# petabi/petal-neighbors

Hardware: AMD Instinct MI355X
Metric: exact k-NN queries/sec (1M x 128 fp32, k=10) (higher is better)
Workload: dtype f32; 1 GPU; c2: 1000000 points x 128 dims f32, 10000 queries, k=10, uniform[0,1); n_points=1000000, dim=128, n_queries=10000, k=10, engine=bf16, exchange=none (one shard), rccl_world_size=1

## Files before the change

### petal-neighbors_amd/csrc/bf16_filter.hip

```cpp
#include "pn_internal.h"
#include "topk_buffer.h"

namespace pn {

typedef __bf16 bf16x8 __attribute__((ext_vector_type(8)));
typedef float f32x16 __attribute__((ext_vector_type(16)));
typedef uint32_t u32x4 __attribute__((ext_vector_type(4)));
typedef __attribute__((address_space(3))) void lds_void_b;
typedef const __attribute__((address_space(1))) void glb_void_b;

#ifdef PN_DIAG_BF_COUNT
__device__ unsigned long long g_bfdbg[16];
#define BF_COUNT(i, v) (dbg_[i] += (unsigned long long)(v))
#define BF_DBG_DECL unsigned long long dbg_[12] = {0, 0, 0, 0, 0, 0, 0, 0, 0, 0, 0, 0}
#define BF_DBG_ARG , unsigned long long (&dbg_)[12]
#define BF_DBG_PASS , dbg_
#define BF_DBG_FLUSH(lane)                                                        \
    do {                                                                          \
        if ((lane) == 0)                                                          \
            for (int i_ = 0; i_ < 12; ++i_) {                                     \
                atomicAdd(&g_bfdbg[i_], dbg_[i_]);                                \
                dbg_[i_] = 0;                                                     \
            }                                                                     \
    } while (0)
__device__ __forceinline__ unsigned long long bf_stamp() {
    unsigned long long t;
    asm volatile("s_memtime %0\n\ts_waitcnt lgkmcnt(0)" : "=s"(t)::"memory");
    return t;
}
__device__ __forceinline__ unsigned long long bf_stamp_nw() {
    unsigned long long t;
    asm volatile("s_memtime %0" : "=s"(t));
    return t;
}
__device__ __forceinline__ void bf_settle(unsigned long long &t) { asm volatile("s_waitcnt lgkmcnt(0)" : "+s"(t)::"memory"); }
#else
#define BF_COUNT(i, v) ((void)0)
#define BF_DBG_DECL ((void)0)
#define BF_DBG_ARG
#define BF_DBG_PASS
#define BF_DBG_FLUSH(lane) ((void)0)
#endif

constexpr int kBQ = 256;
constexpr int kBP = 64;
constexpr double kG = 1.0 / 8192.0;
constexpr double kUp = 1.0 + 1.0 / 1099511627776.0;
__host__ __device__ inline int bf16_extra_col(int dim) {
    const int room = (dim + 15) / 16 * 16 - dim;
    return room >= 5 && dim > 16 ? dim : (dim + 15) / 16 * 16;
}
__host__ __device__ inline int bf16_steps(int dim) { return (bf16_extra_col(dim) + 5 + 15) / 16; }
__host__ __device__ inline bool bf16_ci_dim(int dim) { return dim >= 17 && dim <= 128 && bf16_steps(dim) > (dim + 15) / 16; }
__host__ __device__ inline int bf16_steps_for(int dim, bool ci) { return ci ? (dim + 15) / 16 : bf16_steps(dim); }
// ... 708 lines not shown
    const float a = lo3(l0, l1, l2), am = md3(l0, l1, l2);
    const float b = lo3(l3, l4, l5), bm = md3(l3, l4, l5);
    mn = fminf(a, b);
    const float sec_lo = lo3(fmaxf(a, b), am, bm);
    const float dmin = fminf(lo3(d0, d1, d2), fminf(d3, d4));
    sec = fminf(sec_lo, dmin);
    (void)big;
}

template <int KS, bool CI>
__device__ __forceinline__ void bf_chain(const char *arow, const bf16x8 (&pre)[kLA], const bf16x8 (&b0)[KS],
                                         const bf16x8 (&b1)[KS], const f32x16 &c0, f32x16 &w0, f32x16 &w1, f32x16 &r0,
                                         f32x16 &r1, float &m0, float &m1) {
    bf16x8 f[KS];
#pragma unroll
    for (int i = 0; i < kLA && i < KS; ++i) f[i] = pre[i];
    f32x16 z;
#pragma unroll
    for (int i = 0; i < 16; ++i) z[i] = 0.0f;
#pragma unroll
    for (int ks = 0; ks < KS; ++ks) {
        if (ks + kLA < KS) f[ks + kLA] = *reinterpret_cast<const bf16x8 *>(arow + 32 * (ks + kLA));
        if (CI) {
            w0 = __builtin_amdgcn_mfma_f32_32x32x16_bf16(f[ks], b0[ks], ks ? w0 : c0, 0, 0, 0);
            w1 = __builtin_amdgcn_mfma_f32_32x32x16_bf16(f[ks], b1[ks], ks ? w1 : c0, 0, 0, 0);
        } else {
            w0 = __builtin_amdgcn_mfma_f32_32x32x16_bf16(f[ks], b0[ks], ks ? w0 : z, 0, 0, 0);
            w1 = __builtin_amdgcn_mfma_f32_32x32x16_bf16(f[ks], b1[ks], ks ? w1 : z, 0, 0, 0);
        }
#pragma unroll
        for (int i = 16 * ks / KS; i < 16 * (ks + 1) / KS; ++i) {
            m0 = i ? fminf(m0, r0[i]) : r0[0];
            m1 = i ? fminf(m1, r1[i]) : r1[0];
        }
        __builtin_amdgcn_sched_barrier(0);
    }
}

template <int CP>
__device__ __forceinline__ f32x16 bf_cinit(const char *tb, int blk, int h) {
    typedef float f32x4_ __attribute__((ext_vector_type(4)));
    f32x16 c;
#pragma unroll
    for (int g = 0; g < 4; ++g) {
        const f32x4_ v = *reinterpret_cast<const f32x4_ *>(tb + ((blk * 8 + 2 * g + h) * CP + (CP - 1)) * 16);
        c[4 * g + 0] = v[0];
        c[4 * g + 1] = v[1];
        c[4 * g + 2] = v[2];
        c[4 * g + 3] = v[3];
    }
    return c;
}

template <int KS, bool CI, int CP>
__device__ __forceinline__ void bf_chain_p(const char *arow, bf16x8 (&pre)[kLA], const bf16x8 (&b0)[KS],
                                           const bf16x8 (&b1)[KS], f32x16 &c, f32x16 &w0, f32x16 &w1, f32x16 &r0,
                                           f32x16 &r1, float &m0, float &m1, const char *narow, const char *ntb,
                                           int nblk, int h) {
    typedef float f32x4_ __attribute__((ext_vector_type(4)));
    bf16x8 f[KS];
#pragma unroll
    for (int i = 0; i < kLA && i < KS; ++i) f[i] = pre[i];
    f32x16 z, nc = c;
#pragma unroll
    for (int i = 0; i < 16; ++i) z[i] = 0.0f;
#pragma unroll
    for (int ks = 0; ks < KS; ++ks) {
        if (ks + kLA < KS) f[ks + kLA] = *reinterpret_cast<const bf16x8 *>(arow + 32 * (ks + kLA));
#pragma unroll
        for (int i = 0; i < kLA; ++i)
            if (ks == (KS - kLA + i > 0 ? KS - kLA + i : 0))
                pre[i] = *reinterpret_cast<const bf16x8 *>(narow + 32 * (i < KS ? i : 0));
        if (CI) {
#pragma unroll
            for (int g = 0; g < 4; ++g)
                if (ks == (KS - 4 + g > 0 ? KS - 4 + g : 0)) {
                    const f32x4_ v =
                        *reinterpret_cast<const f32x4_ *>(ntb + ((nblk * 8 + 2 * g + h) * CP + (CP - 1)) * 16);
                    nc[4 * g + 0] = v[0];
                    nc[4 * g + 1] = v[1];
                    nc[4 * g + 2] = v[2];
                    nc[4 * g + 3] = v[3];
                }
            w0 = __builtin_amdgcn_mfma_f32_32x32x16_bf16(f[ks], b0[ks], ks ? w0 : c, 0, 0, 0);
            w1 = __builtin_amdgcn_mfma_f32_32x32x16_bf16(f[ks], b1[ks], ks ? w1 : c, 0, 0, 0);
            if (ks == 0) asm volatile("" ::"v"(c));
        } else {
            w0 = __builtin_amdgcn_mfma_f32_32x32x16_bf16(f[ks], b0[ks], ks ? w0 : z, 0, 0, 0);
            w1 = __builtin_amdgcn_mfma_f32_32x32x16_bf16(f[ks], b1[ks], ks ? w1 : z, 0, 0, 0);
        }
#pragma unroll
        for (int i = 16 * ks / KS; i < 16 * (ks + 1) / KS; ++i) {
            m0 = i ? fminf(m0, r0[i]) : r0[0];
            m1 = i ? fminf(m1, r1[i]) : r1[0];
        }
        __builtin_amdgcn_sched_barrier(0);
    }
    c = nc;
}

constexpr uint32_t kShPeriod = 32;
constexpr uint32_t kShMaxPass = 1u << 14;
__device__ __forceinline__ uint32_t sh_load(const uint32_t *p) {
    return __hip_atomic_load(p, __ATOMIC_RELAXED, __HIP_MEMORY_SCOPE_AGENT);
}
__device__ __forceinline__ void sh_store(uint32_t *p, uint32_t v) {
    __hip_atomic_store(p, v, __ATOMIC_RELAXED, __HIP_MEMORY_SCOPE_AGENT);
}
__device__ __forceinline__ void sh_store_entry(uint2 *p, uint32_t key, uint32_t row) {
    __hip_atomic_store(reinterpret_cast<unsigned long long *>(p), ((unsigned long long)row << 32) | key, __ATOMIC_RELAXED,
                       __HIP_MEMORY_SCOPE_AGENT);
}
__device__ __forceinline__ uint32_t sh_tag(uint32_t epoch, uint32_t ncomp) { return (epoch << 20) | ((ncomp & 0xFFu) << 12); }

template <int M>
__device__ __forceinline__ void bf_refresher(const uint2 *__restrict__ cand, const uint32_t *pcnt, uint32_t *gtau,
                                          const uint32_t *done, uint32_t n_main, size_t nq_pad, uint32_t nseg,
                                          uint32_t epoch, uint32_t rank, uint32_t wv, uint32_t n_wv, int lane) {
    constexpr uint32_t CAP = 64u * M;
    constexpr int NK = 8;
// ... 875 lines not shown
                bf_slow<M, false, SH>(a0, p, tau, cnt, rt * kBP, h, jq, lane, kp, ceq, ce_blk, ns BF_DBG_PASS, pc_blk,
                                      &sh_ncomp, sh.epoch);
            cur = nxt;
        }
        if (SH) {
            if (g_pending) tau = fminf(tau, s2f(g0));
        }
        {
            float m = a1[0];
#pragma unroll
            for (int i = 1; i < 16; ++i) m = fminf(m, a1[i]);
            if (__any(m < tau))
                bf_slow<M, false, SH>(a1, m, tau, cnt, (rt1 - 1) * kBP + 32, h, jq, lane, kp, ceq, ce_blk, ns BF_DBG_PASS,
                                      pc_blk, &sh_ncomp, sh.epoch);
            if (SH) {
                if (h == 0) sh_store(pc_blk + jq, sh_tag(sh.epoch, sh_ncomp + 1u));
            }
        }
        asm volatile("s_waitcnt vmcnt(0)" ::: "memory");
        const uint32_t kfin = keep_arg > kp ? keep_arg : kp;
        unsigned long long need = __ballot(h == 0 && cnt > kfin);
        constexpr int NB = M == 1 ? 4 : 1;
        while (need) {
            int jj[NB];
            uint32_t cj[NB], key[NB][M], ixs[NB][M];
#pragma unroll
            for (int bb = 0; bb < NB; ++bb) {
                jj[bb] = need ? __builtin_ctzll(need) : -1;
                if (need) need &= need - 1;
                cj[bb] = jj[bb] >= 0 ? (uint32_t)__builtin_amdgcn_readlane((int)cnt, jj[bb] >= 0 ? jj[bb] : 0) : 0u;
                if (jj[bb] >= 0) bf_compact_load<M>(ce_blk + (size_t)jj[bb] * CAP, cj[bb], lane, key[bb], ixs[bb]);
            }
#pragma unroll
            for (int bb = 0; bb < NB; ++bb) {
                if (jj[bb] >= 0) {
                    uint32_t T, nn;
                    bf_compact_finish<M>(ce_blk + (size_t)jj[bb] * CAP, key[bb], ixs[bb], cj[bb], kp, lane, T, nn);
                    if (jq == jj[bb]) { tau = fminf(tau, s2f(T)); cnt = nn; }
                }
            }
        }
        if (h == 0) {
            ccnt[cell0 + jq] = cnt;
            ctau[cell0 + jq] = f2s(tau);
        }
        BF_DBG_FLUSH(lane);
    }
    if (SH) {
        __syncthreads();
        if (tid == 0) (void)__hip_atomic_fetch_add(sh.done, 1u, __ATOMIC_RELAXED, __HIP_MEMORY_SCOPE_AGENT);
    }
}

template <int M, bool RAD>
__global__ __launch_bounds__(512, 1) void bf16_wide_kernel(const char *__restrict__ img, uint32_t n_tiles,
                                                           const char *__restrict__ Bimg, uint32_t nkc,
                                                           uint32_t tile_bytes, uint32_t has_x, uint32_t kp,
                                                           uint2 *__restrict__ cand, uint32_t *__restrict__ ccnt,
                                                           uint32_t *__restrict__ ctau, size_t nq_pad,
                                                           uint32_t scout_max,
                                                           const uint32_t *__restrict__ tau_init,
                                                           float *__restrict__ scout_out) {
    constexpr uint32_t CAP = 64u * M;
    extern __shared__ __attribute__((aligned(16))) unsigned char smem_raw[];
    char *lds = reinterpret_cast<char *>(smem_raw);

    const int tid = threadIdx.x, lane = tid & 63;
    const int wave = __builtin_amdgcn_readfirstlane(tid >> 6);
    const int jq = lane & 31, h = lane >> 5;
    const int qg = wave & 3, rh = wave >> 2;
    BF_DBG_DECL;

    uint32_t w = blockIdx.x;
    const uint32_t W = gridDim.x;
    {
        const uint32_t x = blockIdx.x & 7u, base = W >> 3, rem = W & 7u;
        w = x * base + (x < rem ? x : rem) + (blockIdx.x >> 3);
    }
    const unsigned long long U = (unsigned long long)(nq_pad / kWR) * n_tiles, Wn = W;
    unsigned long long u0 = (unsigned long long)w * U / Wn;
    const unsigned long long u1 = (unsigned long long)(w + 1) * U / Wn;
    const float inf = __uint_as_float(0x7F800000u);

    int slot_off[4];
#pragma unroll
    for (int s = 0; s < 4; ++s) slot_off[s] = (int)(((unsigned)(2 * s + h) ^ bf_wide_swz((size_t)jq)) * 16u);
    int st = 0;
    uint32_t ns = 0;
    f32x16 acc[4][2];

    while (u0 < u1) {
    const uint32_t qt = (uint32_t)(u0 / n_tiles);
    const unsigned long long v_begin = (unsigned long long)qt * n_tiles, v_end = v_begin + n_tiles;
    const unsigned long long run_end = u1 < v_end ? u1 : v_end;
    const uint32_t rt0 = (uint32_t)(u0 - v_begin), rt1 = (uint32_t)(run_end - v_begin);
    unsigned long long wf = v_begin * Wn / U;
    while ((wf + 1) * U / Wn <= v_begin) ++wf;
    while (wf > 0 && wf * U / Wn > v_begin) --wf;
    const uint32_t sg = (uint32_t)(w - wf);
    const size_t q0 = (size_t)qt * kWR + (size_t)qg * 64;
    const size_t cell0 = (size_t)(sg * 2 + rh) * nq_pad + q0;
    float tau0 = inf, tau1 = inf;
    uint32_t cnt0 = 0, cnt1 = 0;

    const bool is_a = wave < 4;
    const char *src0 = (is_a ? img : Bimg + (size_t)qt * tile_bytes) + (size_t)(wave & 3) * (kWDma * 1024) + lane * 16;
// ... 414 lines not shown
    if (smp) sm = *smp;
    if (sm.seed_out && (!sm.m1 || !sm.a || !sm.b)) return hipErrorInvalidValue;
    if (!bf16_is_wide(dim)) {
        hipLaunchKernelGGL(bf16_pack_queries8_kernel<T>, dim3((unsigned)(nq_pad * 8 / 256)), dim3(256), 0, s, Q, mu, nq,
                           nq_pad, dim, ld, bf16_ks_for(dim, ci), static_cast<uint16_t *>(B), qn, qbad, ci ? 1 : 0,
                           bmax, dmax, Qp, ldq, misc, sm);
        return hipGetLastError();
    }
    if (ci || nq_pad % 32 != 0) return hipErrorInvalidValue;
    hipLaunchKernelGGL((bf16_pack_wide8_kernel<T, true>), dim3((unsigned)(nq_pad * 8 / 256)), dim3(256), 0, s, Q, mu, nq, nq_pad,
                       dim, ld, static_cast<uint16_t *>(B), qn, qbad, (uint32_t *)nullptr, sm);
    return hipGetLastError();
}
template <typename T>
__global__ void bf16_column_moments_kernel(const T *__restrict__ P, const float *__restrict__ mu, size_t n, int dim, size_t ld,
                                           double *__restrict__ out) {
    const size_t r0 = (size_t)blockIdx.x * 1024;
    const size_t r1 = r0 + 1024 < n ? r0 + 1024 : n;
    for (int k = threadIdx.x; k < dim; k += blockDim.x) {
        const double m = (double)mu[k];
        double s1 = 0.0, s2 = 0.0, s3 = 0.0, s4 = 0.0;
        for (size_t r = r0; r < r1; ++r) {
            const double x = (double)P[r * ld + k];
            const double u = (fabs(x) < 1.0e30) ? x - m : 0.0;
            const double u2 = u * u;
            s1 += u;
            s2 += u2;
            s3 += u2 * u;
            s4 += u2 * u2;
        }
        atomicAdd(&out[k], s1);
        atomicAdd(&out[dim + k], s2);
        atomicAdd(&out[2 * dim + k], s3);
        atomicAdd(&out[3 * dim + k], s4);
    }
}
template <typename T>
hipError_t launch_bf16_column_moments(const T *P, const float *mu, size_t n, int dim, size_t ld, double *out, hipStream_t s) {
    hipLaunchKernelGGL(bf16_column_moments_kernel<T>, dim3((unsigned)((n + 1023) / 1024)), dim3(128), 0, s, P, mu, n, dim, ld, out);
    return hipGetLastError();
}
template hipError_t launch_bf16_column_moments<float>(const float *, const float *, size_t, int, size_t, double *, hipStream_t);
template hipError_t launch_bf16_column_moments<double>(const double *, const float *, size_t, int, size_t, double *, hipStream_t);

template hipError_t launch_bf16_pack_queries<float>(const float *, const float *, size_t, size_t, int, size_t, void *, double *,
                                                    uint32_t *, bool, double, double, hipStream_t, float *, size_t, uint32_t *,
                                                    const Bf16SeedModel *);
template hipError_t launch_bf16_pack_queries<double>(const double *, const float *, size_t, size_t, int, size_t, void *, double *,
                                                     uint32_t *, bool, double, double, hipStream_t, double *, size_t, uint32_t *,
                                                     const Bf16SeedModel *);

constexpr uint32_t kBf8MaxRun = 200;
constexpr size_t kBf8MaxImage = (size_t)768 << 20;
template <int KS, int M, bool RAD, bool CI>
static hipError_t launch_bf16_t(const void *img, uint32_t n_tiles, const void *B, uint32_t q_tiles, uint32_t kp,
                                const CandBuf &cb, int n_wg, uint32_t split, uint32_t spp, uint32_t scout_max,
                                const uint32_t *tau_init, float *scout_out, const Bf16Shared *shp, hipStream_t s) {
    const size_t sh = (size_t)3 * kBP * (2 * KS + 1) * 16 + 16;
    const uint32_t kp_keep = kp | ((uint32_t)(M <= 2 && !RAD && cb.final_keep > (int)kp ? cb.final_keep : 0) << 16);
    const bool use_sh = shp && shp->n_refresh > 0;
    BfShared bsh{};
    bsh.nseg = (uint32_t)cb.nseg;
    if (shp) {
        bsh.seed_lists = shp->seed_lists;
        bsh.seed_rank = shp->seed_rank;
        bsh.seed_nq = shp->seed_nq;
        bsh.seed_words = shp->seed_words;
        if (bsh.seed_lists && (bsh.seed_rank < 1 || bsh.seed_rank > (uint32_t)kScoutList || !bf16_seed_in_kernel(cb.nseg)))
            return hipErrorInvalidValue;
    }
#define PN_BF_LAUNCH_MODE(MD)                                                                                          \
    {                                                                                                                   \
        auto kern = bf16_filter_kernel<KS, M, RAD, CI, MD>;                                                             \
        static LdsAttrOnce lds_attr;                                                             \
        const hipError_t e = lds_attr.ensure(reinterpret_cast<const void *>(kern), sh);                                 \
        if (e != hipSuccess) return e;                                                                                  \
        hipLaunchKernelGGL(kern, dim3((unsigned)n_wg), dim3(256), sh, s, static_cast<const char *>(img), n_tiles,       \
                           static_cast<const u32x4 *>(B), q_tiles, kp_keep, static_cast<uint2 *>(cb.keys), cb.cnt,      \
                           static_cast<uint32_t *>(cb.tau), cb.nq_pad, split, spp, scout_max, tau_init, scout_out,      \
                           bsh);                                                                                        \
    }
    if constexpr (M <= 4 && !RAD) {
        const bool aligned = split == 1 && (uint32_t)n_wg >= q_tiles && (uint32_t)n_wg % q_tiles == 0;
        const uint32_t run_tiles = aligned ? n_tiles / ((uint32_t)n_wg / q_tiles) : 0u;
        const size_t image_bytes = (size_t)n_tiles * kBP * (2 * KS + 1) * 16;
        const bool want8 = cb.bf16_waves == 8 || (cb.bf16_waves == 0 && image_bytes <= kBf8MaxImage &&
                                                  (M >= 2 || run_tiles < kBf8MaxRun));
        if (want8 && aligned && !scout_out && (tau_init || bsh.seed_lists)) {
            if (use_sh && (!tau_init || shp->n_refresh < 1 || M > 2)) return hipErrorInvalidValue;
            BfShared a = bsh;
            if (use_sh) {
                a.pcnt = shp->pcnt;
                a.done = shp->done;
                a.n_main = (uint32_t)n_wg;
                a.epoch = shp->epoch;
                a.rank = shp->rank;
            }
            const unsigned grid = (unsigned)(n_wg + (use_sh ? shp->n_refresh : 0));
#define PN_BF_LAUNCH8(SHV)                                                                                              \
    {                                                                                                                   \
        auto kern = bf16_filter8_kernel<KS, CI, SHV, M>;                                                                  \
        static LdsAttrOnce lds_attr;                                                             \
        const hipError_t e = lds_attr.ensure(reinterpret_cast<const void *>(kern), sh);                                 \
        if (e != hipSuccess) return e;                                                                                  \
        hipLaunchKernelGGL(kern, dim3(grid), dim3(512), sh, s, static_cast<const char *>(img), n_tiles,                 \
                           static_cast<const u32x4 *>(B), q_tiles, kp_keep, static_cast<uint2 *>(cb.keys), cb.cnt,      \
                           static_cast<uint32_t *>(cb.tau), cb.nq_pad, tau_init, a);                                    \
    }
            if (use_sh) PN_BF_LAUNCH8(true) else PN_BF_LAUNCH8(false)
#undef PN_BF_LAUNCH8
            return hipGetLastError();
        }
    }
    if (use_sh) {
        if constexpr (!RAD && M <= 2) {
            if (!tau_init || scout_out || split != 1 || shp->n_refresh < 1) return hipErrorInvalidValue;
            auto kern = bf16_filter_kernel<KS, M, false, CI, 2, true>;
            static LdsAttrOnce lds_attr;
            const hipError_t e = lds_attr.ensure(reinterpret_cast<const void *>(kern), sh);
            if (e != hipSuccess) return e;
            BfShared a = bsh;
            a.pcnt = shp->pcnt;
            a.done = shp->done;
            a.n_main = (uint32_t)n_wg;
            a.epoch = shp->epoch;
            a.rank = shp->rank;
            hipLaunchKernelGGL(kern, dim3((unsigned)(n_wg + shp->n_refresh)), dim3(256), sh, s,
                               static_cast<const char *>(img), n_tiles, static_cast<const u32x4 *>(B), q_tiles, kp_keep,
                               static_cast<uint2 *>(cb.keys), cb.cnt, static_cast<uint32_t *>(cb.tau), cb.nq_pad, split,
                               spp, scout_max, tau_init, scout_out, a);
            return hipGetLastError();
        } else {
            return hipErrorInvalidValue;
        }
    }
    if (scout_out) {
        if (RAD) return hipErrorInvalidValue;
        PN_BF_LAUNCH_MODE(1)
    } else if (tau_init) {
        PN_BF_LAUNCH_MODE(2)
    } else {
        if (RAD) return hipErrorInvalidValue;
        PN_BF_LAUNCH_MODE(0)
    }
#undef PN_BF_LAUNCH_MODE
    return hipGetLastError();
}

template <int KS, bool CI>
static hipError_t launch_bf16_m(const void *img, uint32_t n_tiles, const void *B, uint32_t q_tiles, uint32_t kp,
                                const CandBuf &cb, int n_wg, uint32_t split, uint32_t spp, uint32_t scout_max,
                                const uint32_t *tau_init, bool radius, float *scout_out, const Bf16Shared *shp,
                                hipStream_t s) {
    if (radius)
        return cb.cap == 256 && tau_init && !(shp && shp->n_refresh > 0) ? launch_bf16_t<KS, 4, true, CI>(img, n_tiles, B, q_tiles, kp, cb, n_wg,
                                                                                  split, spp, scout_max, tau_init,
                                                                                  nullptr, nullptr, s)
                                                 : hipErrorInvalidValue;
    switch (cb.cap) {
        case 64:
            return launch_bf16_t<KS, 1, false, CI>(img, n_tiles, B, q_tiles, kp, cb, n_wg, split, spp, scout_max,
                                                   tau_init, scout_out, shp, s);
        case 128:
            return launch_bf16_t<KS, 2, false, CI>(img, n_tiles, B, q_tiles, kp, cb, n_wg, split, spp, scout_max,
                                                   tau_init, scout_out, shp, s);
        case 256:
            return launch_bf16_t<KS, 4, false, CI>(img, n_tiles, B, q_tiles, kp, cb, n_wg, split, spp, scout_max,
                                                   tau_init, scout_out, shp, s);
        default: return hipErrorInvalidValue;
    }
}

int bf16_segments(size_t q_tiles, int n_wg, int split) {
    return split * mfma_v2_max_segments(q_tiles * (size_t)split, n_wg);
}

bool bf16_shared_supported(int cap) {
    return cap == 64 || cap == 128;
}
hipError_t launch_bf16_filter(const void *img, size_t n, int dim, const void *B, int kp, const CandBuf &cb, int n_wg,
                              int split, int scout_max, const uint32_t *tau_init, bool radius, float *scout_out,
                              bool ci, hipStream_t s, const Bf16Shared *shp) {
    if (!bf16_supported(dim) || bf16_is_wide(dim) || cb.nq_pad % kBQ || kp < 1 || kp + 32 > cb.cap || cb.idx_stride != 2 ||
        cb.idx != static_cast<uint32_t *>(cb.keys) + 1 || split < 1 || scout_max < 0 || (ci && !bf16_ci_dim(dim)))
        return hipErrorInvalidValue;
    const uint32_t n_tiles = (uint32_t)((n + kBP - 1) / kBP);
    const uint32_t q_tiles = (uint32_t)(cb.nq_pad / kBQ);
    if ((uint32_t)split > n_tiles) return hipErrorInvalidValue;
    if (shp && shp->n_refresh > 0 &&
        (!(split == 1 && (uint32_t)n_wg >= q_tiles && (uint32_t)n_wg % q_tiles == 0) || !bf16_shared_supported(cb.cap) ||
                shp->epoch < 1 || shp->epoch > 4095 || shp->rank < 1 || !shp->pcnt || !shp->done))
        return hipErrorInvalidValue;
// ... 276 lines not shown
```

### petal-neighbors_amd/csrc/index.hip

```cpp
#include <algorithm>
#include <cmath>
#include <cstdarg>
#include <cstddef>
#include <cstdio>
#include <cstdlib>
#include <cstring>
#include <atomic>
#include <chrono>
#include <mutex>
#include <new>
#include <string>
#include <thread>
#include <vector>

#include "../../include/petal_mi355x.h"
#include "pn_internal.h"

using namespace pn;

static thread_local std::string g_err;

static int fail(int code, const char *fmt, ...) {
    char buf[512];
    va_list ap;
// ... 809 lines not shown
        r->pending = false;
    }
};

extern "C" int pn_index_info(const pn_index *ix, pn_info *out) {
    if (!ix || !out) return fail(PN_ERR_INVALID, "NULL argument");
    out->n_points = ix->n;
    out->dim = ix->dim;
    out->row_stride_device = ix->ld;
    out->elem_bytes = ix->elem_bytes;
    out->device = ix->device;
    out->mfma_eligible = ix->mfma_ok ? 1 : 0;
    out->bf16_eligible = ix->bf16_ok ? 1 : 0;
    out->bf16_layout = !ix->bf16_ok ? 0 : ix->bf16_ci ? 2 : 1;
    out->seed_model = ix->sm_ok ? 1 : 0;
    return PN_OK;
}

extern "C" int pn_index_set_option(pn_index *ix, int option, int64_t value) {
    if (!ix) return fail(PN_ERR_INVALID, "index is NULL");
    std::lock_guard<std::mutex> lk(ix->sh.mu);
    switch (option) {
        case PN_OPT_ENGINE:
            if (value < PN_ENGINE_AUTO || value > PN_ENGINE_BF16) return fail(PN_ERR_INVALID, "bad engine %lld", (long long)value);
            if (ix->metric == 1 && value == PN_ENGINE_MFMA)
                return fail(PN_ERR_UNSUPPORTED, "a Cosine index is served by the bf16 filter or the exact scan");
            if (value == PN_ENGINE_BF16 && !ix->bf16_ok)
                return fail(PN_ERR_UNSUPPORTED, "the bf16 filter cannot serve this index (D > 4096, fewer than 64 rows or out-of-range values)");
            if (value == PN_ENGINE_MFMA && !ix->mfma_ok)
                return fail(PN_ERR_UNSUPPORTED, "the MFMA filter cannot serve this index (f64, non-finite norms or unsupported shape)");
            ix->engine = (int)value;
            ix->sh.bf16_level = 0;
            return PN_OK;
        case PN_OPT_SEGMENTS:
            if (value < 0 || value > 4096) return fail(PN_ERR_INVALID, "bad segment count");
            ix->opt_segments = (int)value;
            return PN_OK;
        case PN_OPT_INDEX_BASE: ix->index_base = (uint64_t)value; return PN_OK;
        case PN_OPT_PROFILE: ix->profile = value < 0 ? 0 : value > 2 ? 2 : (int)value; return PN_OK;
        case PN_OPT_FILTER_SLOTS:
            if (value < 0 || value > 960) return fail(PN_ERR_INVALID, "bad filter slot count");
            ix->filter_slots = (int)value;
            return PN_OK;
        case PN_OPT_MFMA_STRUCTURE:
            if (value == 1) return fail(PN_ERR_INVALID, "structure 1 (the (query tile x segment) grid) was retired in round 4");
            if (value < 0 || value > 3) return fail(PN_ERR_INVALID, "bad structure");
            ix->mfma_structure = (int)value;
            return PN_OK;
        case PN_OPT_SHARED_THRESHOLDS:
            if (value < 0 || value > 4096) return fail(PN_ERR_INVALID, "bad shared-threshold rank");
            ix->shared_tau = (int)value;
            return PN_OK;
        case PN_OPT_BF16_WAVES:
            if (value != 0 && value != 4 && value != 8) return fail(PN_ERR_INVALID, "bad wave count (0, 4 or 8)");
            ix->bf16_waves = (int)value;
            return PN_OK;
        case PN_OPT_SEED_MODEL:
            if (value != 0 && value != 1) return fail(PN_ERR_INVALID, "bad seed-model switch (0 or 1)");
            ix->seed_model = (int)value;
            return PN_OK;
        case PN_OPT_DBSCAN_PIECE:
            if (value < 0) return fail(PN_ERR_INVALID, "bad DBSCAN piece size");
            ix->dbscan_piece = (uint64_t)value;
            return PN_OK;
        case PN_OPT_MST_BATCH:
            if (value < 0) return fail(PN_ERR_INVALID, "bad MST batch size");
            ix->mst_batch = (uint64_t)value;
            return PN_OK;
        case PN_OPT_OPTICS_PIECE:
            if (value < 0) return fail(PN_ERR_INVALID, "bad OPTICS piece size");
            ix->optics_piece = (uint64_t)value;
            return PN_OK;
        case PN_OPT_KDE_PIECE:
            if (value < 0) return fail(PN_ERR_INVALID, "bad KDE piece size");
            ix->kde_piece = (uint64_t)value;
            return PN_OK;
        case PN_OPT_MS_PIECE:
            if (value < 0) return fail(PN_ERR_INVALID, "bad mean shift piece size");
            ix->ms_piece = (uint64_t)value;
            return PN_OK;
        default: return fail(PN_ERR_INVALID, "unknown option %d", option);
    }
}

extern "C" int pn_index_get_stats(const pn_index *ix, pn_stats *out, int reset) {
    if (!ix || !out) return fail(PN_ERR_INVALID, "NULL argument");
    DeviceGuard g(ix->device);
    if (!g.ok) return fail(PN_ERR_DEVICE, "hipSetDevice(%d) failed", ix->device);
    handle_wait(ix, false);
    std::lock_guard<std::mutex> lk(ix->sh.mu);
    recs_collect(ix, true);
    unsigned long long h[kPnStatWords] = {0};
    if (ix->d_stats) HIPCHK(hipMemcpy(h, ix->d_stats, sizeof h, hipMemcpyDeviceToHost));
    *out = ix->sh.stats;
    out->fallback_queries += h[0];
    for (int i = 0; i < kPnStatSlots; ++i) {
        out->candidates += h[4 + 2 * i];
        out->evaluations += h[5 + 2 * i];
    }
    if (reset) {
        ix->sh.stats = pn_stats{};
        if (ix->d_stats) HIPCHK(hipMemset(ix->d_stats, 0, sizeof h));
    }
    return PN_OK;
}

static int pick_cap(size_t kp) {
// ... 761 lines not shown
}

template <typename T>
static int run_bf16(const pn_index *ix, Workspace &ws, const Bf16Plan &plan, const T *Qp, size_t nq, size_t nq_pad,
                    size_t kout, uint64_t *d_idx, T *d_dist, size_t out_stride, hipStream_t s, CallRec *rec,
                    const T *d_q_raw = nullptr, size_t q_stride = 0, const T *qnorm = nullptr) {
    if (!plan.ok) return fail(PN_ERR_UNSUPPORTED, "bf16 tier cannot serve k = %zu", kout);
    const bool cosine = ix->metric == 1;
    if (cosine && (!qnorm || d_q_raw)) return fail(PN_ERR_INVALID, "Cosine tier: query norms missing");
    const int n_wg = plan.n_wg, cap = plan.cap, nseg = plan.nseg;
    const size_t kp = (size_t)plan.kp;
    const size_t cells = (size_t)nseg * nq_pad, slots = cells * (size_t)cap;
    PNCHK(ws.w_bq.ensure(bf16_query_bytes(nq_pad, (int)ix->dim, ix->bf16_ci)));
    PNCHK(ws.w_qn.ensure(nq_pad * sizeof(double)));
    PNCHK(ws.w_qbad.ensure(nq_pad * sizeof(uint32_t)));
    PNCHK(ws.w_keys.ensure(slots * 2 * sizeof(uint32_t)));
    PNCHK(ws.w_cnt.ensure(cells * sizeof(uint32_t)));
    PNCHK(ws.w_tau.ensure(cells * sizeof(uint32_t)));
    PNCHK(ws.w_flags.ensure(nq_pad * sizeof(uint32_t)));
    PNCHK(ws.w_gsel.ensure(nq_pad * sizeof(uint32_t)));
    uint32_t *d_misc = (uint32_t *)ws.w_misc.p;
    const bool model = plan.model_seed && ix->d_smodel;
    Bf16SeedModel smd{};
    if (model) {
        PNCHK(ws.w_seed.ensure(nq_pad * sizeof(uint32_t)));
        smd.m1 = ix->d_smodel;
        smd.a = ix->d_smodel + ix->ld;
        smd.b = ix->d_smodel + 2 * ix->ld;
        smd.c0 = ix->sm_c0;
        smd.v0 = ix->sm_v0;
        smd.z = plan.model_z;
        smd.seed_out = (uint32_t *)ws.w_seed.p;
        if (rec) rec->model_seed = true;
    }
    if (cosine) {
        PNCHK(ws.w_qnrm.ensure(nq_pad * ix->ld * sizeof(double)));
        HIPCHK(launch_cos_normalize_rows<T>(Qp, nq, nq_pad, (int)ix->dim, ix->ld, (double *)ws.w_qnrm.p, ix->ld, nullptr,
                                            true, s));
        HIPCHK(launch_bf16_pack_queries<double>((const double *)ws.w_qnrm.p, ix->d_mu, nq, nq_pad, (int)ix->dim, ix->ld,
                                                ws.w_bq.p, (double *)ws.w_qn.p, (uint32_t *)ws.w_qbad.p, ix->bf16_ci,
                                                ix->bf16_bmax, ix->bf16_dmax, s, (double *)nullptr, 0, nullptr,
                                                model ? &smd : nullptr));
    } else if (d_q_raw)
        HIPCHK(launch_bf16_pack_queries(d_q_raw, ix->d_mu, nq, nq_pad, (int)ix->dim, q_stride, ws.w_bq.p,
                                        (double *)ws.w_qn.p, (uint32_t *)ws.w_qbad.p, ix->bf16_ci, ix->bf16_bmax,
                                        ix->bf16_dmax, s, const_cast<T *>(Qp), ix->ld, d_misc, model ? &smd : nullptr));
    else
        HIPCHK(launch_bf16_pack_queries(Qp, ix->d_mu, nq, nq_pad, (int)ix->dim, ix->ld, ws.w_bq.p, (double *)ws.w_qn.p,
                                        (uint32_t *)ws.w_qbad.p, ix->bf16_ci, ix->bf16_bmax, ix->bf16_dmax, s,
                                        (T *)nullptr, 0, nullptr, model ? &smd : nullptr));
    CandBuf cb{ws.w_keys.p, (uint32_t *)ws.w_keys.p + 1, (uint32_t *)ws.w_cnt.p, ws.w_tau.p, nq_pad, nseg, cap, 2};
    cb.final_keep = bf16_cell_max((int)kp, cap, nseg, bf16_is_wide((int)ix->dim));
    cb.bf16_waves = ix->bf16_waves;
    if (!plan.aligned) {
        HIPCHK(hipMemsetAsync(ws.w_cnt.p, 0, cells * sizeof(uint32_t), s));
        HIPCHK(hipMemsetD32Async((hipDeviceptr_t)ws.w_tau.p, (int)0xFF800000u, cells, s));
    }
    const bool prof = rec && rec->prof;
    if (prof) {
        HIPCHK(hipEventRecord(rec->ev[0], s));
        rec->hot = true;
        rec->two_launches = plan.shared_scout && !model;
    }
    if (plan.shared_scout) {
        const size_t words = cells * 2 * (size_t)bf16_scout_list();
        PNCHK(ws.w_lists.ensure(words * sizeof(float)));
        PNCHK(ws.w_seed.ensure(nq_pad * sizeof(uint32_t)));
        if (!plan.aligned)
            HIPCHK(hipMemsetD32Async((hipDeviceptr_t)ws.w_lists.p, (int)0x7F800000u, words, s));
        if (plan.wide && !model)
            HIPCHK(launch_bf16_wide_filter(ix->d_img, ix->n, (int)ix->dim, ws.w_bq.p, (int)kp, cb, plan.n_wg,
                                           plan.scout_tiles, nullptr, false, (float *)ws.w_lists.p, s));
        const bool seed_in_kernel = !model && !plan.wide && bf16_seed_in_kernel(nseg) && plan.seed_rank <= bf16_scout_list();
        Bf16Shared seed{};
        if (seed_in_kernel) {
            seed.seed_lists = (const float *)ws.w_lists.p;
            seed.seed_rank = (uint32_t)plan.seed_rank;
            seed.seed_nq = (uint32_t)nq;
            seed.seed_words = (uint32_t *)ws.w_seed.p;
        }
        if (!plan.wide && !model)
            HIPCHK(launch_bf16_filter(ix->d_img, ix->n, (int)ix->dim, ws.w_bq.p, (int)kp, cb, n_wg, 1, plan.scout_tiles,
                                      nullptr, false, (float *)ws.w_lists.p, ix->bf16_ci, s,
                                      seed_in_kernel && plan.n_refresh > 0 ? &seed : nullptr));
        if (!seed_in_kernel && !model)
            HIPCHK(launch_bf16_seed((const float *)ws.w_lists.p, nq_pad, nseg, plan.seed_rank, (uint32_t *)ws.w_seed.p, s, nq));
        if (plan.wide)
            HIPCHK(launch_bf16_wide_filter(ix->d_img, ix->n, (int)ix->dim, ws.w_bq.p, (int)kp, cb, plan.n_wg, 0,
                                           (const uint32_t *)ws.w_seed.p, false, nullptr, s));
        else if (plan.n_refresh > 0) {
            const void *pc_before = ws.w_pcnt.p;
            PNCHK(ws.w_pcnt.ensure(cells * sizeof(uint32_t)));
            if (ws.w_pcnt.p != pc_before) ws.sh_nseg = 0;
            if (ws.sh_nseg != (size_t)nseg || ws.sh_nq_pad != nq_pad) {
                HIPCHK(hipMemsetAsync(ws.w_pcnt.p, 0, cells * sizeof(uint32_t), s));
                ws.sh_nseg = (size_t)nseg;
                ws.sh_nq_pad = nq_pad;
            }
            ws.sh_epoch = ws.sh_epoch % 4095u + 1u;
            Bf16Shared shp = seed;
            shp.pcnt = (uint32_t *)ws.w_pcnt.p;
            shp.done = d_misc + 8;
            shp.epoch = ws.sh_epoch;
            shp.rank = (uint32_t)plan.sh_rank;
            shp.n_refresh = plan.n_refresh;
            HIPCHK(launch_bf16_filter(ix->d_img, ix->n, (int)ix->dim, ws.w_bq.p, (int)kp, cb, n_wg, 1, 0,
// ... 3126 lines not shown
```

### petal-neighbors_amd/csrc/pn_internal.h

```cpp
#pragma once
#include <hip/hip_runtime.h>

#include <atomic>
#include <cstddef>
#include <cstdint>
#include <type_traits>

namespace pn {

struct LdsAttrOnce {
    std::atomic<uint64_t> done{0};
    hipError_t ensure(const void *kern, size_t bytes) {
        int dev = 0;
        hipError_t e = hipGetDevice(&dev);
        if (e != hipSuccess) return e;
        const uint64_t bit = 1ull << (dev & 63);
        if (done.load(std::memory_order_acquire) & bit) return hipSuccess;
        e = hipFuncSetAttribute(kern, hipFuncAttributeMaxDynamicSharedMemorySize, (int)bytes);
        if (e == hipSuccess) done.fetch_or(bit, std::memory_order_release);
        return e;
    }
};

constexpr int kTileQ = 64;
constexpr int kTileP = 64;
constexpr int kChunkK = 32;
constexpr int kRowAlign = 8;
constexpr int kRowPad = 256;

template <typename T> struct KeyOf;
template <> struct KeyOf<float> {
    using type = uint32_t;
    static constexpr type kMax = 0xFFFFFFFFu;
    static constexpr type kNaN = 0x7FC00000u;
};
template <> struct KeyOf<double> {
    using type = uint64_t;
    static constexpr type kMax = 0xFFFFFFFFFFFFFFFFull;
    static constexpr type kNaN = 0x7FF8000000000000ull;
};

struct CandBuf {
    void *keys;
    uint32_t *idx;
    uint32_t *cnt;
    void *tau;
    size_t nq_pad;
    int nseg;
    int cap;
    int idx_stride = 1;
    int final_keep = 0;
    int bf16_waves = 0;
};

inline size_t round_up(size_t a, size_t b) { return (a + b - 1) / b * b; }

hipError_t launch_exact_knn_f32(const float *P, size_t n, int dim, size_t ldp, const float *Q, int nq,
                                size_t ldq, int kp, size_t seg_len, const CandBuf &cb, const void *lo_key,
                                const uint32_t *lo_idx, const uint32_t *nq_dev, uint32_t nq_off, const float *pnorm,
                                const float *qnorm, hipStream_t s, const uint32_t *qsel = nullptr);
hipError_t launch_exact_knn_f64(const double *P, size_t n, int dim, size_t ldp, const double *Q, int nq,
                                size_t ldq, int kp, size_t seg_len, const CandBuf &cb, const void *lo_key,
                                const uint32_t *lo_idx, const uint32_t *nq_dev, uint32_t nq_off, const double *pnorm,
                                const double *qnorm, hipStream_t s, const uint32_t *qsel = nullptr);
hipError_t launch_exact_radius_f32(const float *P, size_t n, int dim, size_t ldp, const float *Q, int nq,
                                   size_t ldq, float r, size_t seg_len, int nseg, uint32_t *counts,
                                   const uint64_t *offsets, uint64_t *fill, uint64_t index_base, const float *pnorm,
                                   const float *qnorm, hipStream_t s, const uint32_t *qsel = nullptr,
                                   const uint32_t *nq_dev = nullptr, uint64_t capacity = ~0ull,
                                   float *fill_dist = nullptr, const float *radii = nullptr);
hipError_t launch_exact_radius_f64(const double *P, size_t n, int dim, size_t ldp, const double *Q, int nq,
                                   size_t ldq, double r, size_t seg_len, int nseg, uint32_t *counts,
                                   const uint64_t *offsets, uint64_t *fill, uint64_t index_base, const double *pnorm,
                                   const double *qnorm, hipStream_t s, const uint32_t *qsel = nullptr,
                                   const uint32_t *nq_dev = nullptr, uint64_t capacity = ~0ull,
                                   double *fill_dist = nullptr, const double *radii = nullptr);

hipError_t launch_rad_list(const uint32_t *over, const uint32_t *bad, int nq, uint32_t *nkept, uint32_t *sel,
                           uint32_t *pos, uint32_t *nsel, hipStream_t s);
hipError_t launch_rad_counts(const uint32_t *nkept, const uint32_t *pos, const uint32_t *counts_x, int nseg, int nq,
                             uint32_t *fin, hipStream_t s);
hipError_t launch_exclusive_scan_u32(const uint32_t *in, size_t n, uint64_t *offsets, uint64_t *scratch, uint64_t *total,
                                     hipStream_t s);
hipError_t launch_rad_seg_offsets(const uint64_t *offsets, const uint32_t *sel, const uint32_t *nsel, int nq,
                                  const uint32_t *counts_x, int nseg, uint64_t *offs_x, hipStream_t s);
hipError_t launch_radius_gather_cap(const uint32_t *kept, const uint32_t *nkept, const uint64_t *offsets, int nq,
                                    size_t kept_stride, uint64_t index_base, uint64_t *out, uint64_t capacity,
                                    hipStream_t s, const void *kept_dist = nullptr, void *out_dist = nullptr,
                                    int dist_bytes = 0);

hipError_t launch_knn_self_exclude_f32(const uint64_t *in_idx, const float *in_dist, size_t nq, int kin, int kout,
                                       uint64_t self0, uint64_t *out_idx, float *out_dist, hipStream_t s);
hipError_t launch_knn_self_exclude_f64(const uint64_t *in_idx, const double *in_dist, size_t nq, int kin, int kout,
                                       uint64_t self0, uint64_t *out_idx, double *out_dist, hipStream_t s);
hipError_t launch_radius_self_counts_f32(const float *P, size_t n, int dim, size_t ld, const float *cnorm, float r,
                                         bool exclude, const uint64_t *in_off, uint32_t *flag, uint32_t *cnt, uint32_t *bad,
                                         hipStream_t s, const float *radii = nullptr);
hipError_t launch_radius_self_counts_f64(const double *P, size_t n, int dim, size_t ld, const double *cnorm, double r,
                                         bool exclude, const uint64_t *in_off, uint32_t *flag, uint32_t *cnt, uint32_t *bad,
                                         hipStream_t s, const double *radii = nullptr);
hipError_t launch_radius_self_place(const uint64_t *part, size_t nq, uint64_t *out, hipStream_t s);
hipError_t launch_radius_self_compact_f32(const uint64_t *in_off, const uint64_t *in_idx, const float *in_dist,
                                          uint64_t in_cap, const uint32_t *flag, const uint64_t *out_off, size_t n,
                                          uint64_t self0, uint64_t *out_idx, float *out_dist, uint64_t cap, uint32_t *bad,
                                          hipStream_t s);
// ... 362 lines not shown
```

Baseline: 4.990 million queries/s.

## Add paired-query-tile bf16 filter kernel sharing one point-tile stream across eight waves

Adds a new bf16 filter kernel in which one 512-thread workgroup serves two query tiles. The point tiles are streamed into a triple-buffered LDS ring by all eight waves, so each point tile fetched from global memory is reused by twice as many queries. The second half of the waves meets the DMA barrier mid-chain (staggered) so its MFMA work overlaps with the first half's sync and loads. The kernel is auto-selected for M=1 aligned runs with long per-workgroup runs when the grid fills the CU slots, in place of the 8-wave kernel. This brings more complex barrier scheduling and a risk of occupancy or LDS limits.

```diff
diff --git a/petal-neighbors_amd/csrc/bf16_filter.hip b/petal-neighbors_amd/csrc/bf16_filter.hip
--- a/petal-neighbors_amd/csrc/bf16_filter.hip
+++ b/petal-neighbors_amd/csrc/bf16_filter.hip
@@ -1,5 +1,8 @@
 #include "pn_internal.h"
 #include "topk_buffer.h"
+
+#include <cstdio>
+#include <cstdlib>
 
 namespace pn {
 
@@ -814,11 +817,15 @@
     return c;
 }
 
-template <int KS, bool CI, int CP>
+struct BfNoMid {
+    static constexpr int at(int) { return -1; }
+    __device__ __forceinline__ void operator()() const {}
+};
+template <int KS, bool CI, int CP, typename MID = BfNoMid>
 __device__ __forceinline__ void bf_chain_p(const char *arow, bf16x8 (&pre)[kLA], const bf16x8 (&b0)[KS],
                                            const bf16x8 (&b1)[KS], f32x16 &c, f32x16 &w0, f32x16 &w1, f32x16 &r0,
                                            f32x16 &r1, float &m0, float &m1, const char *narow, const char *ntb,
-                                           int nblk, int h) {
+                                           int nblk, int h, MID mid = MID()) {
     typedef float f32x4_ __attribute__((ext_vector_type(4)));
     bf16x8 f[KS];
 #pragma unroll
@@ -828,6 +835,7 @@
     for (int i = 0; i < 16; ++i) z[i] = 0.0f;
 #pragma unroll
     for (int ks = 0; ks < KS; ++ks) {
+        if (ks == MID::at(KS)) mid();
         if (ks + kLA < KS) f[ks + kLA] = *reinterpret_cast<const bf16x8 *>(arow + 32 * (ks + kLA));
 #pragma unroll
         for (int i = 0; i < kLA; ++i)
@@ -1809,6 +1817,240 @@
     }
 }
 
+#ifndef PN_DIAG_PAIR_STAGGER
+#define PN_DIAG_PAIR_STAGGER 1
+#endif
+constexpr int kPairStagger = PN_DIAG_PAIR_STAGGER;
+#ifndef PN_DIAG_PAIR_MID4
+#define PN_DIAG_PAIR_MID4 2
+#endif
+struct BfPairMeet {
+    uint32_t ns;
+    static constexpr int at(int ks) { return ks * PN_DIAG_PAIR_MID4 / 4 > 1 ? ks * PN_DIAG_PAIR_MID4 / 4 : 1; }
+    __device__ __forceinline__ void operator()() const {
+        bf_wait_dma(ns);
+        __builtin_amdgcn_s_barrier();
+        asm volatile("" ::: "memory");
+    }
+};
+
+template <int KS, bool CI, int STAG>
+__device__ __forceinline__ void bf_pair_run(const char *__restrict__ img, char *tiles, uint32_t kp, uint32_t kfin, uint2 *__restrict__ cand,
+                                            uint32_t *__restrict__ ccnt, uint32_t *__restrict__ ctau,
+                                            const bf16x8 (&b0)[KS], const bf16x8 (&b1)[KS], float tau0, float tau1,
+                                            uint32_t rt0, uint32_t rt1, size_t cell0, bool active, int wave, int lane) {
+    constexpr int C = 2 * KS, CP = C + 1;
+    constexpr uint32_t CAP = 64u;
+    constexpr int TB = kBP * CP * 16;
+    constexpr int NBUF = 3, NW = 8;
+    const int jq = lane & 31, h = lane >> 5;
+    BF_DBG_DECL;
+    constexpr int P = (CP + NW - 1) / NW;
+    static_assert(P <= 3, "piece schedule written out for up to three pieces per wave");
+    const int n_mine = CP - wave * P < P ? (CP - wave * P > 0 ? CP - wave * P : 0) : P;
+    const uint32_t lane_off = (uint32_t)lane * 16u;
+    auto dma_tile = [&](uint32_t rt, int buf) {
+        const char *wbase = img + ((size_t)rt * (size_t)TB + (size_t)(wave * (P * 1024)));
+        const char *ws = wbase + lane_off;
+        char *wd = tiles + buf * TB + wave * (P * 1024);
+        if (0 < n_mine) __builtin_amdgcn_global_load_lds((glb_void_b *)ws, (lds_void_b *)wd, 16, 0, 0);
+        if (P > 1 && 1 < n_mine) __builtin_amdgcn_global_load_lds((glb_void_b *)ws, (lds_void_b *)wd, 16, 1024, 0);
+        if (P > 2 && 2 < n_mine) __builtin_amdgcn_global_load_lds((glb_void_b *)ws, (lds_void_b *)wd, 16, 2048, 0);
+    };
+
+    uint32_t cnt0 = 0, cnt1 = 0;
+    uint2 *ce_blk0 = cand + cell0 * CAP;
+    uint2 *ce_blk1 = ce_blk0 + (size_t)32 * CAP;
+    uint2 *ceq0 = ce_blk0 + (size_t)jq * CAP, *ceq1 = ce_blk1 + (size_t)jq * CAP;
+    uint32_t ns = 0;
+
+    f32x16 a00, a01, a10, a11;
+#pragma unroll
+    for (int r = 0; r < 16; ++r) {
+        a00[r] = 3.0e38f;
+        a01[r] = 3.0e38f;
+        a10[r] = 3.0e38f;
+        a11[r] = 3.0e38f;
+    }
+    bf16x8 pre[kLA];
+    f32x16 cc = a00;
+    {
+        const char *ar = tiles + (jq * CP + h) * 16;
+#pragma unroll
+        for (int i = 0; i < kLA; ++i) pre[i] = *reinterpret_cast<const bf16x8 *>(ar + 32 * (i < KS ? i : 0));
+        if (CI) cc = bf_cinit<CP>(tiles, 0, h);
+    }
+    int cur = 0;
+    for (uint32_t rt = rt0; rt < rt1; ++rt) {
+        const int nxt = cur == NBUF - 1 ? 0 : cur + 1, prv = cur == 0 ? NBUF - 1 : cur - 1;
+        const char *tb = tiles + cur * TB;
+        const char *arow0 = tb + (jq * CP + h) * 16;
+        const char *arow1 = arow0 + 32 * CP * 16;
+        float m0, m1, p0, p1;
+        if (STAG == 2) BfPairMeet{ns}();
+        if (STAG == 1)
+            bf_chain_p<KS, CI, CP>(arow0, pre, b0, b1, cc, a00, a01, a10, a11, m0, m1, arow1, tb, 1, h, BfPairMeet{ns});
+        else
+            bf_chain_p<KS, CI, CP>(arow0, pre, b0, b1, cc, a00, a01, a10, a11, m0, m1, arow1, tb, 1, h);
+        if (rt == rt0) { m0 = __uint_as_float(0x7F800000u); m1 = m0; }
+        if (__any(m0 < tau0 || m1 < tau1)) {
+            const uint32_t row0 = (rt - 1) * kBP + 32;
+            if (__any(m0 < tau0)) bf_slow<1, false>(a10, m0, tau0, cnt0, row0, h, jq, lane, kp, ceq0, ce_blk0, ns BF_DBG_PASS);
+            if (__any(m1 < tau1)) bf_slow<1, false>(a11, m1, tau1, cnt1, row0, h, jq, lane, kp, ceq1, ce_blk1, ns BF_DBG_PASS);
+        }
+        if (STAG == 0) {
+            bf_wait_dma(ns);
+#ifndef PN_DIAG_PAIR_NOLGKM
+            asm volatile("s_waitcnt lgkmcnt(0)" ::: "memory");
+#endif
+            __builtin_amdgcn_s_barrier();
+            asm volatile("" ::: "memory");
+        }
+        if (rt + 2 < rt1) {
+            dma_tile(rt + 2, prv);
+            ns = 0;
+        }
+        const bool last = rt + 1 >= rt1;
+        const char *ntb = last ? tb : tiles + nxt * TB;
+        bf_chain_p<KS, CI, CP>(arow1, pre, b0, b1, cc, a10, a11, a00, a01, p0, p1, ntb + (jq * CP + h) * 16, ntb, 0, h);
+        if (__any(p0 < tau0 || p1 < tau1)) {
+            const uint32_t row0 = rt * kBP;
+            if (__any(p0 < tau0)) bf_slow<1, false>(a00, p0, tau0, cnt0, row0, h, jq, lane, kp, ceq0, ce_blk0, ns BF_DBG_PASS);
+            if (__any(p1 < tau1)) bf_slow<1, false>(a01, p1, tau1, cnt1, row0, h, jq, lane, kp, ceq1, ce_blk1, ns BF_DBG_PASS);
+        }
+        cur = nxt;
+    }
+    {
+        float m0 = a10[0], m1 = a11[0];
+#pragma unroll
+        for (int i = 1; i < 16; ++i) {
+            m0 = fminf(m0, a10[i]);
+            m1 = fminf(m1, a11[i]);
+        }
+        const uint32_t row0 = (rt1 - 1) * kBP + 32;
+        if (__any(m0 < tau0)) bf_slow<1, false>(a10, m0, tau0, cnt0, row0, h, jq, lane, kp, ceq0, ce_blk0, ns BF_DBG_PASS);
+        if (__any(m1 < tau1)) bf_slow<1, false>(a11, m1, tau1, cnt1, row0, h, jq, lane, kp, ceq1, ce_blk1, ns BF_DBG_PASS);
+    }
+    asm volatile("s_waitcnt vmcnt(0)" ::: "memory");
+    auto final_compact = [&](uint2 *ce_blk, float &tau, uint32_t &cnt) {
+        constexpr int NB = 4;
+        unsigned long long need = __ballot(h == 0 && cnt > kfin);
+        while (need) {
+            int jj[NB];
+            uint32_t cj[NB], key[NB][1], ixs[NB][1];
+#pragma unroll
+            for (int b = 0; b < NB; ++b) {
+                jj[b] = need ? __builtin_ctzll(need) : -1;
+                if (need) need &= need - 1;
+                cj[b] = jj[b] >= 0 ? (uint32_t)__builtin_amdgcn_readlane((int)cnt, jj[b] >= 0 ? jj[b] : 0) : 0u;
+                if (jj[b] >= 0) bf_compact_load<1>(ce_blk + (size_t)jj[b] * CAP, cj[b], lane, key[b], ixs[b]);
+            }
+#pragma unroll
+            for (int b = 0; b < NB; ++b) {
+                if (jj[b] >= 0) {
+                    uint32_t T, nn;
+                    bf_compact_finish<1>(ce_blk + (size_t)jj[b] * CAP, key[b], ixs[b], cj[b], kp, lane, T, nn);
+                    if (jq == jj[b]) { tau = fminf(tau, s2f(T)); cnt = nn; }
+                }
+            }
+        }
+    };
+    final_compact(ce_blk0, tau0, cnt0);
+    final_compact(ce_blk1, tau1, cnt1);
+    if (active && h == 0) {
+        ccnt[cell0 + jq] = cnt0;
+        ctau[cell0 + jq] = f2s(tau0);
+        ccnt[cell0 + 32 + jq] = cnt1;
+        ctau[cell0 + 32 + jq] = f2s(tau1);
+    }
+    BF_DBG_FLUSH(lane);
+}
+
+template <int KS, bool CI>
+__global__ __launch_bounds__(512, 2) void bf16_filter_kernel_pair(const char *__restrict__ img, uint32_t n_tiles,
+                                                                  const u32x4 *__restrict__ Bq, uint32_t q_tiles,
+                                                                  uint32_t kp_keep, uint2 *__restrict__ cand,
+                                                                  uint32_t *__restrict__ ccnt,
+                                                                  uint32_t *__restrict__ ctau, size_t nq_pad,
+                                                                  const uint32_t *tau_init, BfShared sh) {
+    const uint32_t kp = kp_keep & 0xFFFFu, keep_arg = kp_keep >> 16;
+    const uint32_t kfin = keep_arg > kp ? keep_arg : kp;
+    constexpr int CP = 2 * KS + 1;
+    constexpr int TB = kBP * CP * 16;
+    extern __shared__ __attribute__((aligned(16))) unsigned char smem_raw[];
+    char *tiles = reinterpret_cast<char *>(smem_raw);
+    const int tid = threadIdx.x, lane = tid & 63;
+    const int wave = __builtin_amdgcn_readfirstlane(tid >> 6);
+    const int jq = lane & 31, h = lane >> 5;
+    constexpr int C = 2 * KS;
+    const uint32_t W = gridDim.x, n_pairs = (q_tiles + 1u) >> 1, c_per = W / n_pairs;
+    uint32_t w;
+    {
+        const uint32_t b = blockIdx.x, x = b & 7u, base = W >> 3, rem = W & 7u;
+        const uint32_t L = x * base + (x < rem ? x : rem) + (b >> 3);
+        w = (L % n_pairs) * c_per + L / n_pairs;
+    }
+    const uint32_t pt = w / c_per, seg = w % c_per;
+    const uint32_t rt0 = (uint32_t)((unsigned long long)seg * n_tiles / c_per);
+    const uint32_t rt1 = (uint32_t)((unsigned long long)(seg + 1) * n_tiles / c_per);
+    if (rt0 >= rt1) return;
+    const uint32_t qt = 2u * pt + (uint32_t)(wave >> 2);
+    const bool active = qt < q_tiles;
+    const size_t q0 = active ? (size_t)qt * kBQ + (size_t)(wave & 3) * 64 : 0;
+    const size_t cell0 = (size_t)seg * nq_pad + q0;
+
+    bf16x8 b0[KS], b1[KS];
+    float tau0 = __uint_as_float(0xFF800000u), tau1 = tau0;
+    if (active) {
+        const u32x4 *br0 = Bq + (q0 + jq) * (size_t)C + h;
+        const u32x4 *br1 = br0 + (size_t)32 * C;
+#pragma unroll
+        for (int ks = 0; ks < KS; ++ks) {
+            const u32x4 v0 = br0[2 * ks], v1 = br1[2 * ks];
+            b0[ks] = __builtin_bit_cast(bf16x8, v0);
+            b1[ks] = __builtin_bit_cast(bf16x8, v1);
+        }
+        if (sh.seed_lists) {
+            const size_t ql = q0 + (size_t)lane;
+            float sd = __uint_as_float(0xFF800000u);
+            if (ql < (size_t)sh.seed_nq) {
+                const uint32_t key = f2s(bf_seed_lane(sh.seed_lists, nq_pad, sh.nseg, sh.seed_rank, ql));
+                sd = s2f(key == 0xFFFFFFFFu ? key : key + 1u);
+            }
+            tau0 = __shfl(sd, jq);
+            tau1 = __shfl(sd, 32 + jq);
+        } else {
+            tau0 = s2f(tau_init[q0 + jq]);
+            tau1 = s2f(tau_init[q0 + 32 + jq]);
+        }
+    } else {
+        const u32x4 zero = {0u, 0u, 0u, 0u};
+#pragma unroll
+        for (int ks = 0; ks < KS; ++ks) {
+            b0[ks] = __builtin_bit_cast(bf16x8, zero);
+            b1[ks] = b0[ks];
+        }
+    }
+    {
+        constexpr int P = (CP + 7) / 8;
+        const int n_mine = CP - wave * P < P ? (CP - wave * P > 0 ? CP - wave * P : 0) : P;
+        for (uint32_t t = 0; t < 2u && rt0 + t < rt1; ++t) {
+            const char *ws = img + ((size_t)(rt0 + t) * (size_t)TB + (size_t)(wave * (P * 1024))) + (uint32_t)lane * 16u;
+            char *wd = tiles + t * TB + wave * (P * 1024);
+            if (0 < n_mine) __builtin_amdgcn_global_load_lds((glb_void_b *)ws, (lds_void_b *)wd, 16, 0, 0);
+            if (P > 1 && 1 < n_mine) __builtin_amdgcn_global_load_lds((glb_void_b *)ws, (lds_void_b *)wd, 16, 1024, 0);
+            if (P > 2 && 2 < n_mine) __builtin_amdgcn_global_load_lds((glb_void_b *)ws, (lds_void_b *)wd, 16, 2048, 0);
+        }
+    }
+    __syncthreads();
+    if (wave >= 4)
+        bf_pair_run<KS, CI, kPairStagger>(img, tiles, kp, kfin, cand, ccnt, ctau, b0, b1, tau0, tau1, rt0, rt1, cell0,
+                                          active, wave, lane);
+    else
+        bf_pair_run<KS, CI, 0>(img, tiles, kp, kfin, cand, ccnt, ctau, b0, b1, tau0, tau1, rt0, rt1, cell0, active, wave,
+                               lane);
+}
+
 template <int M, bool RAD>
 __global__ __launch_bounds__(512, 1) void bf16_wide_kernel(const char *__restrict__ img, uint32_t n_tiles,
                                                            const char *__restrict__ Bimg, uint32_t nkc,
@@ -2329,6 +2571,15 @@
 
 constexpr uint32_t kBf8MaxRun = 200;
 constexpr size_t kBf8MaxImage = (size_t)768 << 20;
+constexpr bool kPairAuto = true;
+#ifndef PN_DIAG_PAIR_MIN_RUN
+#define PN_DIAG_PAIR_MIN_RUN 200
+#endif
+constexpr uint32_t kPairMinRun = PN_DIAG_PAIR_MIN_RUN;
+static void bf_debug_kernel(const char *which, unsigned grid, unsigned block) {
+    static const bool on = getenv("PN_DEBUG_PLAN") != nullptr;
+    if (on) std::fprintf(stderr, "bf16 main pass: kernel %s grid %u x %u\n", which, grid, block);
+}
 template <int KS, int M, bool RAD, bool CI>
 static hipError_t launch_bf16_t(const void *img, uint32_t n_tiles, const void *B, uint32_t q_tiles, uint32_t kp,
                                 const CandBuf &cb, int n_wg, uint32_t split, uint32_t spp, uint32_t scout_max,
@@ -2361,6 +2612,24 @@
         const bool aligned = split == 1 && (uint32_t)n_wg >= q_tiles && (uint32_t)n_wg % q_tiles == 0;
         const uint32_t run_tiles = aligned ? n_tiles / ((uint32_t)n_wg / q_tiles) : 0u;
         const size_t image_bytes = (size_t)n_tiles * kBP * (2 * KS + 1) * 16;
+        if constexpr (M == 1) {
+            const bool can_pair = aligned && !scout_out && (tau_init || bsh.seed_lists) && !use_sh && q_tiles >= 2;
+            const bool fills = cb.wg_slots > 0 && n_wg >= cb.wg_slots;
+            const bool want_pair = cb.bf16_waves == 16 || (cb.bf16_waves == 0 && kPairAuto && fills &&
+                                                           run_tiles >= kPairMinRun && image_bytes <= kBf8MaxImage);
+            if (want_pair && can_pair) {
+                const unsigned grid = (unsigned)(((q_tiles + 1u) / 2u) * ((uint32_t)n_wg / q_tiles));
+                auto kern = bf16_filter_kernel_pair<KS, CI>;
+                static LdsAttrOnce lds_attr;
+                const hipError_t e = lds_attr.ensure(reinterpret_cast<const void *>(kern), sh);
+                if (e != hipSuccess) return e;
+                bf_debug_kernel("pair", grid, 512);
+                hipLaunchKernelGGL(kern, dim3(grid), dim3(512), sh, s, static_cast<const char *>(img), n_tiles,
+                                   static_cast<const u32x4 *>(B), q_tiles, kp_keep, static_cast<uint2 *>(cb.keys), cb.cnt,
+                                   static_cast<uint32_t *>(cb.tau), cb.nq_pad, tau_init, bsh);
+                return hipGetLastError();
+            }
+        }
         const bool want8 = cb.bf16_waves == 8 || (cb.bf16_waves == 0 && image_bytes <= kBf8MaxImage &&
                                                   (M >= 2 || run_tiles < kBf8MaxRun));
         if (want8 && aligned && !scout_out && (tau_init || bsh.seed_lists)) {
@@ -2384,6 +2653,7 @@
                            static_cast<const u32x4 *>(B), q_tiles, kp_keep, static_cast<uint2 *>(cb.keys), cb.cnt,      \
                            static_cast<uint32_t *>(cb.tau), cb.nq_pad, tau_init, a);                                    \
     }
+            bf_debug_kernel("8", grid, 512);
             if (use_sh) PN_BF_LAUNCH8(true) else PN_BF_LAUNCH8(false)
 #undef PN_BF_LAUNCH8
             return hipGetLastError();
@@ -2402,6 +2672,7 @@
             a.n_main = (uint32_t)n_wg;
             a.epoch = shp->epoch;
             a.rank = shp->rank;
+            bf_debug_kernel("4", (unsigned)(n_wg + shp->n_refresh), 256);
             hipLaunchKernelGGL(kern, dim3((unsigned)(n_wg + shp->n_refresh)), dim3(256), sh, s,
                                static_cast<const char *>(img), n_tiles, static_cast<const u32x4 *>(B), q_tiles, kp_keep,
                                static_cast<uint2 *>(cb.keys), cb.cnt, static_cast<uint32_t *>(cb.tau), cb.nq_pad, split,
@@ -2415,6 +2686,7 @@
         if (RAD) return hipErrorInvalidValue;
         PN_BF_LAUNCH_MODE(1)
     } else if (tau_init) {
+        if (!RAD) bf_debug_kernel("4", (unsigned)n_wg, 256);
         PN_BF_LAUNCH_MODE(2)
     } else {
         if (RAD) return hipErrorInvalidValue;
diff --git a/petal-neighbors_amd/csrc/index.hip b/petal-neighbors_amd/csrc/index.hip
--- a/petal-neighbors_amd/csrc/index.hip
+++ b/petal-neighbors_amd/csrc/index.hip
@@ -885,7 +885,7 @@
             ix->shared_tau = (int)value;
             return PN_OK;
         case PN_OPT_BF16_WAVES:
-            if (value != 0 && value != 4 && value != 8) return fail(PN_ERR_INVALID, "bad wave count (0, 4 or 8)");
+            if (value != 0 && value != 4 && value != 8 && value != 16) return fail(PN_ERR_INVALID, "bad wave count (0, 4, 8 or 16)");
             ix->bf16_waves = (int)value;
             return PN_OK;
         case PN_OPT_SEED_MODEL:
@@ -1753,6 +1753,7 @@
     CandBuf cb{ws.w_keys.p, (uint32_t *)ws.w_keys.p + 1, (uint32_t *)ws.w_cnt.p, ws.w_tau.p, nq_pad, nseg, cap, 2};
     cb.final_keep = bf16_cell_max((int)kp, cap, nseg, bf16_is_wide((int)ix->dim));
     cb.bf16_waves = ix->bf16_waves;
+    cb.wg_slots = 2 * ix->n_cu;
     if (!plan.aligned) {
         HIPCHK(hipMemsetAsync(ws.w_cnt.p, 0, cells * sizeof(uint32_t), s));
         HIPCHK(hipMemsetD32Async((hipDeviceptr_t)ws.w_tau.p, (int)0xFF800000u, cells, s));
diff --git a/petal-neighbors_amd/csrc/pn_internal.h b/petal-neighbors_amd/csrc/pn_internal.h
--- a/petal-neighbors_amd/csrc/pn_internal.h
+++ b/petal-neighbors_amd/csrc/pn_internal.h
@@ -51,6 +51,7 @@
     int idx_stride = 1;
     int final_keep = 0;
     int bf16_waves = 0;
+    int wg_slots = 0;
 };
 
 inline size_t round_up(size_t a, size_t b) { return (a + b - 1) / b * b; }
```

Measured after the change: 5.193 million queries/s (median of 6 runs). 4.1% higher.
